# zendesk/min-tfs-client

Measured on NVIDIA H100. Metric: TensorProto encode+decode GB/s, higher is better.
Workload: dtype u8

## Files before the change

### min-tfs-client_b200/csrc/codec_host.cpp

```cpp
#include <cuda_runtime.h>
#include <stdarg.h>
#include <stdio.h>
#include <stdlib.h>
#include <string.h>

#include <algorithm>
#include <string>
#include <unordered_map>
#include <vector>

#include "../../include/b200tfs.h"
#include "frame.h"
#include "kernels.h"
#include "plan.h"
#include "tpl.h"
#include "walker.h"
#include "wire.h"

using namespace b200tfs;

static thread_local char g_err[512] = "";

static int fail(int code, const char* fmt, ...) {
  va_list ap;
// ... 1095 lines not shown
        else pb.payload(w + r.off, dst + run, bytes, op, r.len, r.stride);
        run += bytes;
      }
      if (pad) {
        if (run % di.elem_size || run > o.dst_bytes) return fail(B200TFS_E_SHAPE, "output %d: %llu value bytes for a tensor of %llu", j,
                                                                  (unsigned long long)run, (unsigned long long)o.dst_bytes);
        fills.push_back(Fill{dst, di.elem_size, run / di.elem_size, o.n_elems});
      }
    } else {
      if (want != o.dtype) return fail(B200TFS_E_DTYPE, "output %d: cast on varint dtypes is not supported", j);
      VarDecodeJob vj{};
      bool plain = runs.size() <= (size_t)B200TFS_MAX_RUNS;
      for (const b200tfs_run& r : runs) plain = plain && r.count == 1;
      if (plain) {
        vj.n_chunks = (int)runs.size();
        for (size_t k = 0; k < runs.size(); ++k) { vj.src[k] = w + runs[k].off; vj.len[k] = runs[k].len; }
      } else {
        gather_cur = (gather_cur + 15) & ~15ull;
        uint8_t* g = (uint8_t*)c->gather_dev.p + gather_cur;
        uint64_t at = 0;
        for (const b200tfs_run& r : runs) {
          const uint64_t bytes = (uint64_t)r.len * r.count;
          if (r.count == 1) pb.payload(w + r.off, g + at, bytes, OP_COPY);
          else pb.payload(w + r.off, g + at, bytes, OP_COPY, r.len, r.stride);
          at += bytes;
        }
        gather_cur += at;
        vj.n_chunks = 1; vj.src[0] = g; vj.len[0] = at;
      }
      vj.dst = dst; vj.n_elems = o.n_elems; vj.dtype = o.dtype; vj.out_index = j; vj.half_as_value = half_as_value; vj.pad_edge = pad;
      vjobs.push_back(vj);
    }
  }
  int rc = launch_plan(c, pb);
  if (rc) return rc;
  for (const Fill& f : fills) { CU(launch_fill_edge(f.dst, f.elem_size, f.have, nullptr, f.n_elems, c->stream)); c->launches += 1; }
  c->pending_status.clear();
  if (!vjobs.empty()) {
    if ((rc = run_vardecode(c, vjobs, status))) return rc;
  }
  if (status && wait) {
    CU(cudaStreamSynchronize(c->stream));
    collect_varint_status(c, status);
  }
  return B200TFS_OK;
}

extern "C" int b200tfs_unpack_outputs(b200tfs_ctx* c, const void* arena_dev, int32_t m, const b200tfs_output* outs,
                                      const uint64_t* out_rec_off, void* const* dst_dev, const int32_t* dst_dtype, int32_t* status) {
  return unpack_outputs_impl(c, arena_dev, m, outs, out_rec_off, dst_dev, dst_dtype, status, true);
}

namespace {
struct FusedLayout { uint64_t outs, nouts, specs, status, vstatus, total; };
FusedLayout fused_layout(int32_t n) {
  FusedLayout L;
  L.outs = 0;
  L.nouts = L.outs + sizeof(b200tfs_output) * (uint64_t)n * kFusedMaxOutputs;
  L.specs = (L.nouts + 4ull * n + 15) & ~15ull;
  L.status = L.specs + sizeof(b200tfs_model_spec) * (uint64_t)n;
  L.vstatus = (L.status + 4ull * n + 15) & ~15ull;
  L.total = (L.vstatus + 4ull * n * kFusedMaxOutputs + 15) & ~15ull;
  return L;
}

struct VarPlanLayout { uint64_t jobs, segs, tile_seg, tile_val, group_sum, total, status, n_tiles, bytes; };
VarPlanLayout var_plan_layout(uint64_t n, uint64_t tile_cap) {
  const uint64_t slots = n * kFusedMaxOutputs;
  VarPlanLayout V;
  V.jobs = 0;
  V.segs = V.jobs + slots * sizeof(VarJobDev);
  V.tile_seg = (V.segs + slots * B200TFS_MAX_RUNS * sizeof(VarSeg) + 15) & ~15ull;
  V.tile_val = (V.tile_seg + 4 * tile_cap + 15) & ~15ull;
  V.group_sum = (V.tile_val + 4 * tile_cap + 15) & ~15ull;
  V.total = (V.group_sum + 4 * (tile_cap / kVarGroupTiles + slots + 2) + 15) & ~15ull;
  V.status = V.total + 8 * slots;
  V.n_tiles = (V.status + 4 * slots + 15) & ~15ull;
  V.bytes = V.n_tiles + 16;
  return V;
}
}

extern "C" {

static void adopt_pinned_template(b200tfs_ctx* c) {
  if (!c->tpl_pinned) return;
  const TplInline& p = *c->tpl_pinned;
  if (p.head.serial && (int32_t)(p.head.serial - c->tpl_known.head.serial) > 0) c->tpl_known = p;
}

static uint32_t decode_vpt(const b200tfs_ctx* c, int32_t n, const uint64_t* rec_len) {
  uint64_t wire_total = 0;
  for (int i = 0; i < n; ++i) wire_total += rec_len[i];
  return pick_vec_per_tile(c, c->decode_cast ? wire_total / 2 : wire_total, c->decode_cast ? 65536 : 262144);
}

static bool host_template(const uint8_t* rec0, uint64_t len, uint32_t vpt, uint64_t dst_stride, uint32_t serial, uint32_t cast, uint32_t varints,
                          Template* T) {
  T->in.head.valid = 0;
  if (!rec0 || len == 0 || len > 0x7FFFFFFFull) return false;
  b200tfs_output outs[kFusedMaxOutputs + 1];
  b200tfs_model_spec spec;
  int cnt = 0;
  Cursor cur;
  cur_open_host(cur, rec0, (uint32_t)len);
  SpillArea sp{nullptr, 0u, 0u};
  const int st = walk_response(cur, kFusedMaxOutputs, outs, &cnt, &spec, sp);
  if (st != B200TFS_OK) return false;
  const uint64_t used = tpl_layout_outputs(outs, cnt, dst_stride, cast, varints);
  for (int k = 0; k < cnt; ++k) if (outs[k].status == B200TFS_E_SIZE) return false;
  tpl_learn(T, cur, (uint32_t)len, outs, cnt, spec, st, vpt, (used + 255) & ~255ull, serial, cast, varints);
  return T->in.head.valid != 0;
}

int b200tfs_decode_slot_bytes(const void* wire_host, int32_t n, const uint64_t* rec_off, const uint64_t* rec_len, int32_t varints,
// ... 28 lines not shown
};

static int decode_launch(b200tfs_ctx* c, const void* arena_dev, int32_t n, const uint64_t* rec_off, const uint64_t* rec_len, void* dst_dev,
                         uint64_t dst_stride, uint32_t vpt, const Template* host_tpl, const DecodeSlices* sl = nullptr) {
  const uint64_t tile_bytes = 16ull * vpt;
  FusedLayout L = fused_layout(n);
  int rc;
  if ((rc = grow_host(c, c->fused_host, L.total))) return rc;
  uint64_t var_tile_cap = 0;
  if (c->decode_varints) {
    for (int i = 0; i < n; ++i) var_tile_cap += var_record_tile_bound(rec_len[i]);
    if (var_tile_cap > 0x7FFFFFFFull) return fail(B200TFS_E_TOOBIG, "batch needs more than 2^31 varint tiles");
    if ((rc = grow_dev(c, c->vdec_dev, var_plan_layout((uint64_t)n, var_tile_cap).bytes))) return rc;
  }
  if (!c->tpl_dev) {
    if (c->capturing) return fail(B200TFS_E_ARG, "run b200tfs_decode_responses once before capturing it");
    CU(cudaMalloc(&c->tpl_dev, 2 * sizeof(Template) + 64));
    CU(cudaMemsetAsync(c->tpl_dev, 0, 2 * sizeof(Template) + 64, c->stream));
    CU(cudaHostAlloc((void**)&c->tpl_pinned, sizeof(TplInline), cudaHostAllocPortable | cudaHostAllocMapped));
    memset(c->tpl_pinned, 0, sizeof(TplInline));
  }
  FusedParams fp{};
  fp.w = (const uint8_t*)arena_dev; fp.dst = (uint8_t*)dst_dev; fp.dst_stride = dst_stride; fp.n = n; fp.vpt = vpt;
  fp.tpl_read = (const Template*)c->tpl_dev + (c->tpl_flip & 1);
  fp.tpl_write = (Template*)c->tpl_dev + ((c->tpl_flip & 1) ^ 1);
  c->tpl_flip ^= 1;
  fp.tpl_pinned = c->tpl_pinned;
  fp.stats = (unsigned long long*)((uint8_t*)c->tpl_dev + 2 * sizeof(Template));
  if (++c->serial == 0) c->serial = 1;
  fp.serial = c->serial;
  fp.cast = c->decode_cast;
  fp.varints = c->decode_varints;
  fp.tpli.head.valid = 0;
  if (host_tpl && host_tpl->in.head.valid) {
    if (vpt <= kStageVecsHost) {
      Slot* slot;
      if ((rc = claim_slot(c, sizeof(Template), &slot))) return rc;
      memcpy(slot->host.p, host_tpl, sizeof(Template));
      CU(cudaMemcpyAsync((void*)fp.tpl_read, slot->host.p, sizeof(Template), cudaMemcpyHostToDevice, c->stream));
      if (slot->done) { CU(cudaEventRecord(slot->done, c->stream)); slot->pending = true; }
      c->tpl_known = host_tpl->in;
      if (!c->opt_no_inline) fp.tpli = host_tpl->in;
    }
  } else {
    if (!c->capturing && (!c->tpl_event_pending || cudaEventQuery(c->tpl_event) == cudaSuccess)) { c->tpl_event_pending = false; adopt_pinned_template(c); }
    const TplHead& h = c->tpl_known.head;
    if (vpt <= kStageVecsHost && !c->opt_no_inline && h.valid && h.rec_len == rec_len[0] && h.vpt == vpt && h.cast == fp.cast &&
        h.varints == fp.varints && h.dst_need <= dst_stride)
      fp.tpli = c->tpl_known;
  }
  const TplHead& kh = (host_tpl && host_tpl->in.head.valid) ? host_tpl->in.head : c->tpl_known.head;
  const bool budget_known = kh.valid && kh.vpt == vpt && kh.cast == fp.cast && kh.varints == fp.varints && kh.dst_need <= dst_stride;
  auto ctas_for = [&](uint64_t len) -> uint64_t {
    if (budget_known && len == kh.rec_len) return (uint64_t)kh.total_tiles + 2;
    return (len + tile_bytes - 1) / tile_bytes + kFusedSlackTiles;
  };
  uint8_t* d = (uint8_t*)c->fused_host.p;
  fp.outs = (b200tfs_output*)(d + L.outs); fp.n_outs = (int32_t*)(d + L.nouts);
  fp.specs = (b200tfs_model_spec*)(d + L.specs); fp.status = (int32_t*)(d + L.status);
  auto lay_out = [&](FusedParams& q, auto&& per, uint64_t* grid_out) -> int {
    uint64_t grid = 0;
    if (n <= kFusedInlineRecs) {
      for (int i = 0; i < n; ++i) {
        q.inl.off[i] = rec_off[i]; q.inl.len[i] = rec_len[i]; q.inl.tile_start[i] = (uint32_t)grid;
        grid += per(rec_len[i]);
      }
      q.inl.tile_start[n] = (uint32_t)grid;
    } else {
      std::vector<uint32_t> ts(n + 1);
      for (int i = 0; i < n; ++i) { ts[i] = (uint32_t)grid; grid += per(rec_len[i]); }
      ts[n] = (uint32_t)grid;
      if (grid > 0x7FFFFFFFull) return fail(B200TFS_E_TOOBIG, "batch needs more than 2^31 tiles");
      const uint64_t o_ts = (grid * 4 + 15) & ~15ull, o_off = (o_ts + 4ull * (n + 1) + 15) & ~15ull, o_len = o_off + 8ull * n;
      const uint64_t image = o_len + 8ull * n;
      Slot* slot;
      int rc2;
      if ((rc2 = claim_slot(c, image, &slot))) return rc2;
      uint8_t* h = (uint8_t*)slot->host.p;
      uint32_t* cr = (uint32_t*)h;
      for (int i = 0; i < n; ++i) for (uint32_t t = ts[i]; t < ts[i + 1]; ++t) cr[t] = (uint32_t)i;
      memcpy(h + o_ts, ts.data(), 4ull * (n + 1));
      memcpy(h + o_off, rec_off, 8ull * n);
      memcpy(h + o_len, rec_len, 8ull * n);
      if ((rc2 = upload_slot(c, slot, image))) return rc2;
      uint8_t* sd = (uint8_t*)slot->dev.p;
      q.cta_rec = (const uint32_t*)sd; q.tile_start = (const uint32_t*)(sd + o_ts);
      q.rec_off = (const uint64_t*)(sd + o_off); q.rec_len = (const uint64_t*)(sd + o_len);
    }
    if (grid > 0x7FFFFFFFull) return fail(B200TFS_E_TOOBIG, "batch needs more than 2^31 tiles");
    *grid_out = grid;
    return B200TFS_OK;
  };
  const TplInline* kt = (host_tpl && host_tpl->in.head.valid) ? &host_tpl->in : &c->tpl_known;
  bool split = fp.cast && !sl && budget_known && kh.total_tiles > 0 && (uint64_t)n * kh.rec_len >= (4ull << 20) && !c->opt_no_inline;
  for (int i = 0; i < n && split; ++i) split = rec_len[i] == kh.rec_len;
  if (split) {
    if ((rc = grow_dev(c, c->guard_dev, 4ull * n))) return rc;
    FusedParams fa = fp;
    fa.mode = 1; fa.guard = (uint32_t*)c->guard_dev.p; fa.tpli = *kt;
    uint64_t ga = 0;
    if ((rc = lay_out(fa, [](uint64_t) -> uint64_t { return 2; }, &ga))) return rc;
    CU(launch_decode_fused(fa, (uint32_t)ga, c->stream));
    PlanBuilder pb;
    uint32_t per_rec = 0;
    for (uint32_t q = 0; q < kt->head.n_chunks; ++q) if (kt->chunk[q].n_tiles) ++per_rec;
    pb.items.reserve((size_t)n * per_rec);
    for (int i = 0; i < n; ++i)
      for (uint32_t q = 0; q < kt->head.n_chunks; ++q) {
        const TplChunk& ch = kt->chunk[q];
        if (!ch.n_tiles) continue;
        const bool narrow = ch.op == OP_F2H || ch.op == OP_F2B;
        const uint64_t n_out = narrow ? ch.len / 2 : ch.len;
        pb.items.push_back(MoveItem{(const uint8_t*)arena_dev + rec_off[i] + ch.wire_off, (uint8_t*)dst_dev + (uint64_t)i * dst_stride + ch.dst_off, n_out,
                                    ch.op, 0, 0, 0});
        pb.large_bytes += n_out;
      }
    pb.guard = (const uint32_t*)c->guard_dev.p; pb.guard_div = per_rec;
    BuiltPlan bp;
    if ((rc = build_plan(c, pb, true, &bp))) return rc;
    CU(launch_move_guarded(bp.plan_dev, bp.ph.n_tiles, c->stream));
    if (bp.slot && bp.slot->done && !c->capturing) { CU(cudaEventRecord(bp.slot->done, c->stream)); bp.slot->pending = true; }
    c->launches += 2;
    fp.mode = 2; fp.guard = (uint32_t*)c->guard_dev.p;
  }
  uint64_t grid = 0;
  if ((rc = lay_out(fp, ctas_for, &grid))) return rc;
  if (sl) {
    if (n != 1 || !fp.tpli.head.valid) return fail(B200TFS_E_ARG, "internal: sliced decode without a host template");
    fp.trusted = 1;
    for (int k = 0; k < sl->K; ++k) {
      CU(cudaStreamWaitEvent(c->stream, sl->before[k], 0));
      fp.tile_bias = sl->tile_lo[k];
      const uint32_t end = (k + 1 == sl->K) ? (uint32_t)grid : sl->tile_lo[k + 1];
      CU(launch_decode_fused(fp, end - sl->tile_lo[k], c->stream));
      CU(cudaEventRecord(sl->after[k], c->stream));
      c->launches += 1;
    }
  } else {
    CU(launch_decode_fused(fp, (uint32_t)grid, c->stream));
    c->launches += 1;
  }
  c->fused_varints = fp.varints != 0;
  if (fp.varints) {
    const VarPlanLayout V = var_plan_layout((uint64_t)n, var_tile_cap);
    uint8_t* vd = (uint8_t*)c->vdec_dev.p;
    VarPlan vp{};
    vp.outs = fp.outs; vp.n_outs = fp.n_outs; vp.rec_status = fp.status;
    vp.w = fp.w; vp.rec_off = fp.rec_off;
    if (n <= kFusedInlineRecs) for (int i = 0; i < n; ++i) vp.off_inl[i] = rec_off[i];
    vp.dst = fp.dst; vp.dst_stride = dst_stride; vp.n = (uint32_t)n; vp.tile_cap = (uint32_t)var_tile_cap;
    vp.jobs = (VarJobDev*)(vd + V.jobs); vp.segs = (VarSeg*)(vd + V.segs); vp.tile_seg = (uint32_t*)(vd + V.tile_seg);
    vp.tile_val = (uint32_t*)(vd + V.tile_val); vp.group_sum = (uint32_t*)(vd + V.group_sum);
    vp.total = (unsigned long long*)(vd + V.total); vp.status = (int32_t*)(vd + V.status); vp.n_tiles = (uint32_t*)(vd + V.n_tiles);
    CU(launch_vdec_plan(vp, c->stream));
    VarTables tb{};
    tb.segs = vp.segs; tb.tile_seg = vp.tile_seg; tb.jobs = vp.jobs; tb.n_tiles = vp.tile_cap; tb.n_tiles_dev = vp.n_tiles;
    CU(launch_vdec_dev(tb, (uint32_t)c->sm_count * 4, c->stream));
    CU(cudaMemcpyAsync((uint8_t*)c->fused_host.p + L.vstatus, vp.status, 4ull * n * kFusedMaxOutputs, cudaMemcpyDeviceToHost, c->stream));
    c->launches += 3;
  }
  c->fused_n = n;
  if (!c->capturing) { CU(cudaEventRecord(c->tpl_event, c->stream)); c->tpl_event_pending = true; }
  return B200TFS_OK;
}

int b200tfs_decode_responses(b200tfs_ctx* c, const void* arena_dev, int32_t n, const uint64_t* rec_off, const uint64_t* rec_len,
                             void* dst_dev, uint64_t dst_stride) {
  if (!c || n < 0 || (n && (!arena_dev || !rec_off || !rec_len || !dst_dev))) return fail(B200TFS_E_ARG, "bad arguments");
  if (n == 0) return B200TFS_OK;
  if (dst_stride & 255) return fail(B200TFS_E_ARG, "dst_stride must be a multiple of 256");
  if (!c->capturing) CU(cudaSetDevice(c->device));
  return decode_launch(c, arena_dev, n, rec_off, rec_len, dst_dev, dst_stride, decode_vpt(c, n, rec_len), nullptr);
}

int b200tfs_set_decode_cast(b200tfs_ctx* c, int32_t float_as) {
  if (!c) return fail(B200TFS_E_ARG, "ctx is NULL");
  if (c->capturing) return fail(B200TFS_E_ARG, "cannot change the decode cast during graph capture");
  if (float_as != 0 && float_as != DT_FLOAT && float_as != DT_HALF && float_as != DT_BFLOAT16)
    return fail(B200TFS_E_DTYPE, "DT_FLOAT outputs can leave as DT_FLOAT, DT_HALF or DT_BFLOAT16, not as dtype %d", float_as);
  c->decode_cast = (float_as == DT_HALF || float_as == DT_BFLOAT16) ? (uint32_t)float_as : 0u;
  return B200TFS_OK;
}

int b200tfs_set_decode_varints(b200tfs_ctx* c, int32_t on) {
  if (!c) return fail(B200TFS_E_ARG, "ctx is NULL");
  if (c->capturing) return fail(B200TFS_E_ARG, "cannot switch the varint decode during graph capture");
  c->decode_varints = on ? 1u : 0u;
  return B200TFS_OK;
}

int b200tfs_decode_results(b200tfs_ctx* c, int32_t n, b200tfs_output* outs, int32_t* n_outs, b200tfs_model_spec* specs,
                           int32_t* rec_status) {
  if (!c || n < 0) return fail(B200TFS_E_ARG, "bad arguments");
  if (c->capturing) return fail(B200TFS_E_ARG, "cannot collect results during graph capture");
  if (n > c->fused_n) return fail(B200TFS_E_ARG, "only %d records were decoded", c->fused_n);
  FusedLayout L = fused_layout(c->fused_n);
  CU(cudaStreamSynchronize(c->stream));
  const uint8_t* h = (const uint8_t*)c->fused_host.p;
  if (outs) memcpy(outs, h + L.outs, sizeof(b200tfs_output) * (uint64_t)n * kFusedMaxOutputs);
  if (outs && c->fused_varints) {
    const int32_t* rs = (const int32_t*)(h + L.status);
    const int32_t* no = (const int32_t*)(h + L.nouts);
    const int32_t* vs = (const int32_t*)(h + L.vstatus);
    for (int r = 0; r < n; ++r)
      for (int k = 0; k < no[r] && rs[r] == B200TFS_OK && k < kFusedMaxOutputs; ++k) {
        b200tfs_output& o = outs[(size_t)r * kFusedMaxOutputs + k];
        const int32_t s = vs[(size_t)r * kFusedMaxOutputs + k];
        if (s == kVarSlotIdle) continue;
        o.status = s;
        o.flags |= B200TFS_OF_DEVICE_VARINT;
      }
  }
  if (n_outs) memcpy(n_outs, h + L.nouts, 4ull * n);
  if (specs) memcpy(specs, h + L.specs, sizeof(b200tfs_model_spec) * (uint64_t)n);
  if (rec_status) memcpy(rec_status, h + L.status, 4ull * n);
  return B200TFS_OK;
}

int b200tfs_decode_stats(b200tfs_ctx* c, uint64_t* param_template, uint64_t* device_template, uint64_t* walked) {
  if (!c) return fail(B200TFS_E_ARG, "ctx is NULL");
  if (c->capturing) return fail(B200TFS_E_ARG, "cannot read the counters during graph capture");
  unsigned long long v[3] = {0, 0, 0};
  if (c->tpl_dev) {
    CU(cudaSetDevice(c->device));
    CU(cudaMemcpyAsync(v, (uint8_t*)c->tpl_dev + 2 * sizeof(Template), sizeof v, cudaMemcpyDeviceToHost, c->stream));
    CU(cudaStreamSynchronize(c->stream));
  }
  if (param_template) *param_template = v[0];
  if (device_template) *device_template = v[1];
  if (walked) *walked = v[2];
  return B200TFS_OK;
}

int b200tfs_capture_begin(b200tfs_ctx* c) {
  if (!c) return fail(B200TFS_E_ARG, "ctx is NULL");
  if (c->capturing) return fail(B200TFS_E_ARG, "already capturing");
  CU(cudaSetDevice(c->device));
  CU(cudaStreamSynchronize(c->stream));
  adopt_pinned_template(c);
  for (auto& s : c->slots) s.pending = false;
  CU(cudaStreamBeginCapture(c->stream, cudaStreamCaptureModeRelaxed));
  c->capturing = true;
  return B200TFS_OK;
}

int b200tfs_capture_end(b200tfs_ctx* c, void** graph_exec) {
  if (!c || !graph_exec) return fail(B200TFS_E_ARG, "NULL argument");
  if (!c->capturing) return fail(B200TFS_E_ARG, "not capturing");
  c->capturing = false;
  cudaGraph_t g = nullptr;
  CU(cudaStreamEndCapture(c->stream, &g));
  cudaGraphExec_t ge = nullptr;
  cudaError_t e = cudaGraphInstantiate(&ge, g, 0);
  cudaGraphDestroy(g);
  if (e != cudaSuccess) return fail(B200TFS_E_CUDA, "cudaGraphInstantiate: %s", cudaGetErrorString(e));
  c->has_graphs = true;
  *graph_exec = ge;
  return B200TFS_OK;
}

int b200tfs_graph_launch(b200tfs_ctx* c, void* graph_exec) {
  if (!c || !graph_exec) return fail(B200TFS_E_ARG, "NULL argument");
  CU(cudaGraphLaunch((cudaGraphExec_t)graph_exec, c->stream));
  return B200TFS_OK;
}

int b200tfs_graph_destroy(void* graph_exec) {
// ... 675 lines not shown
```

### min-tfs-client_b200/csrc/kernels.cu

```cuda
#include <cuda_bf16.h>
#include <cuda_fp16.h>
#include <cuda_runtime.h>
#include <stdint.h>
#include <stdlib.h>
#include <string.h>

#include <algorithm>
#include <utility>

#include "frame.h"
#include "kernels.h"
#include "plan.h"
#include "tpl.h"
#include "walker.h"
#include "wire.h"

namespace b200tfs {

__device__ __forceinline__ uint4 ld_stream(const uint8_t* p) {
  uint4 r;
  asm volatile("ld.global.nc.L1::no_allocate.v4.u32 {%0,%1,%2,%3}, [%4];"
               : "=r"(r.x), "=r"(r.y), "=r"(r.z), "=r"(r.w) : "l"(p));
  return r;
}
// ... 608 lines not shown
  const uint64_t* s = reinterpret_cast<const uint64_t*>(src);
  uint64_t* d = reinterpret_cast<uint64_t*>(dst);
  for (uint32_t i = threadIdx.x; i < bytes / 8; i += blockDim.x) d[i] = s[i];
}

__device__ __noinline__ void fused_slow_path(const FusedParams& fp, uint32_t r, uint32_t j, uint32_t budget, bool publish, const uint8_t* rec,
                                             uint64_t len, uint8_t* dst_slot, uint8_t* lines, b200tfs_output* outs_s, b200tfs_model_spec& spec_s,
                                             FusedJob& job) {
    int cnt = 0, st;
    Cursor c;
    job.valid = 0;
    if (len > 0x7FFFFFFFull) st = B200TFS_E_PARSE;
    else {
      cur_open(c, rec, (uint32_t)len, lines);
      SpillArea sp{nullptr, 0u, 0u};
      st = walk_response(c, kFusedMaxOutputs, outs_s, &cnt, &spec_s, sp);
      if (st == B200TFS_E_SPILL) st = B200TFS_E_NONCANONICAL;
    }
    uint64_t cursor = 0;
    uint32_t t_base = 0;
    if (st == B200TFS_OK) {
      cursor = tpl_layout_outputs(outs_s, cnt, fp.dst_stride, fp.cast, fp.varints);
      uint32_t done_mask[kFusedMaxOutputs] = {0};
      for (;;) {
        int bk = -1, bq = -1; uint64_t best = ~0ull;
        for (int k = 0; k < cnt; ++k) {
          const b200tfs_output& o = outs_s[k];
          if (o.status != B200TFS_OK || !o.n_elems || dtype_info(o.dtype).kind != VK_FIXED) continue;
          for (int q = 0; q < o.n_runs; ++q)
            if (!(done_mask[k] >> q & 1) && o.runs[q].off < best) { best = o.runs[q].off; bk = k; bq = q; }
        }
        if (bk < 0) break;
        done_mask[bk] |= 1u << bq;
        const b200tfs_output& o = outs_s[bk];
        uint64_t run = 0;
        for (int q = 0; q < bq; ++q) run += (uint64_t)o.runs[q].len * o.runs[q].count;
        const b200tfs_run& rn = o.runs[bq];
        const bool narrow = tpl_narrows(fp.cast, o.dtype);
        const uint64_t bytes = ((uint64_t)rn.len * rn.count) >> (narrow ? 1 : 0);
        const uint32_t nt = tiles_for(bytes, fp.vpt);
        if (j >= t_base && j < t_base + nt) {
          job.src = rec + rn.off; job.dst = dst_slot + o.dst_off + (narrow ? run / 2 : run); job.n_out = bytes;
          job.op = tpl_move_op(fp.cast, o.dtype); job.n_tiles = nt; job.tile = j - t_base; job.valid = 1;
          job.glen = rn.count > 1 ? rn.len : 0u; job.gstride = rn.count > 1 ? rn.stride : 0u;
        }
        t_base += nt;
      }
      if (t_base > budget) st = B200TFS_E_NONCANONICAL;
    }
    if (publish) {
      if (fp.stats) atomicAdd(&fp.stats[2], 1ull);
      fp.status[r] = st;
      fp.n_outs[r] = (st == B200TFS_OK) ? cnt : 0;
      fp.specs[r] = spec_s;
      for (int k = 0; k < cnt && st == B200TFS_OK; ++k) fp.outs[(size_t)r * kFusedMaxOutputs + k] = outs_s[k];
      if (r == 0) {
        if (len <= 0x7FFFFFFFull) tpl_learn(fp.tpl_write, c, (uint32_t)len, outs_s, cnt, spec_s, st, fp.vpt, (cursor + 255) & ~255ull, fp.serial, fp.cast,
                                            fp.varints);
        else fp.tpl_write->in.head.valid = 0;
        if (fp.tpl_pinned) {
          fp.tpl_pinned->head.valid = 0;
          __threadfence_system();
          const uint64_t* s8 = reinterpret_cast<const uint64_t*>(&fp.tpl_write->in);
          uint64_t* d8 = reinterpret_cast<uint64_t*>(fp.tpl_pinned);
          const bool ok = fp.tpl_write->in.head.valid != 0;
          if (ok) for (uint32_t q = sizeof(TplHead) / 8; q < sizeof(TplInline) / 8; ++q) d8[q] = s8[q];
          __threadfence_system();
          TplHead h = fp.tpl_write->in.head;
          h.serial = fp.serial; h.valid = ok ? 1u : 0u;
          const uint64_t* h8 = reinterpret_cast<const uint64_t*>(&h);
          for (uint32_t q = sizeof(TplHead) / 8; q-- > 0;) d8[q] = h8[q];
        }
      }
    }
    if (st != B200TFS_OK) job.valid = 0;
}

template <bool STAGED, bool CAST>
__device__ __forceinline__ void decode_fused_body(const FusedParams& fp) {
  pdl_launch_dependents();
  __shared__ __align__(16) uint8_t lines[256];
  __shared__ b200tfs_output outs_s[kFusedMaxOutputs + 1];
  __shared__ b200tfs_model_spec spec_s;
  __shared__ FusedJob job;
  extern __shared__ __align__(128) uint8_t stage_smem[];
  __shared__ __align__(8) uint64_t stage_bars[kStageBufs];
  __shared__ TplChunk ch_s[kTplChunks];
  __shared__ TplHead th_s;
  if (STAGED && threadIdx.x == 0) {
    for (uint32_t q = 0; q < kStageBufs; ++q) mbar_init(&stage_bars[q], 1);
    asm volatile("fence.mbarrier_init.release.cluster;" ::: "memory");
  }
  const uint32_t b = blockIdx.x + fp.tile_bias;
  uint32_t r, j, budget;
  uint64_t off, len;
  if (fp.n <= kFusedInlineRecs) {
    r = 0;
    while (r + 1 < (uint32_t)fp.n && b >= fp.inl.tile_start[r + 1]) ++r;
    j = b - fp.inl.tile_start[r]; off = fp.inl.off[r]; len = fp.inl.len[r];
    budget = fp.inl.tile_start[r + 1] - fp.inl.tile_start[r];
  } else {
    r = fp.cta_rec[b];
    const uint32_t t0 = fp.tile_start[r];
    j = b - t0; off = fp.rec_off[r]; len = fp.rec_len[r];
    budget = fp.tile_start[r + 1] - t0;
  }
  const uint8_t* rec = fp.w + off;
  uint8_t* dst_slot = fp.dst + (uint64_t)r * fp.dst_stride;
  pdl_wait_prior_grids();
  if (CAST && fp.mode == 2 && fp.guard[r] != 0) return;

  const Template* T = fp.tpl_read;
  const bool inl = !STAGED && fp.tpli.head.valid != 0;
  uint32_t live = budget;
  const uint32_t i = threadIdx.x;
  {
    if (inl) {
      if (i < kTplChunks) ch_s[i] = fp.tpli.chunk[i];
      if (i == kTplChunks) th_s = fp.tpli.head;
    } else {
      if (i < kTplChunks) ch_s[i] = T->in.chunk[i];
      if (i == kTplChunks) th_s = T->in.head;
    }
    __syncthreads();
    const uint32_t nch = th_s.n_chunks;
    if (th_s.valid && th_s.rec_len == len && th_s.vpt == fp.vpt && th_s.cast == fp.cast && th_s.varints == fp.varints && th_s.dst_need <= fp.dst_stride &&
        (th_s.total_tiles < budget || (CAST && fp.mode == 1))) {
      auto verdict = [&]() -> bool {
        bool same = true;
        if (!STAGED && fp.trusted && inl) return true;
        if (STAGED) {
          if (i < th_s.framing_len) {
            uint32_t w = i;
            for (uint32_t q = 0; q < nch; ++q) if (ch_s[q].fpos <= i) w += ch_s[q].len;
            same = rec[w] == T->in.framing[i];
          }
          if (i < nch && ch_s[i].is_varint && ch_s[i].len) same = same && !(rec[ch_s[i].wire_off + ch_s[i].len - 1] & 0x80);
          return __syncthreads_and(same) != 0;
        }
        const uint32_t lane = i & 31;
        for (uint32_t k = lane; k < th_s.framing_len; k += 32) {
          uint32_t w = k;
          for (uint32_t q = 0; q < nch; ++q) if (ch_s[q].fpos <= k) w += ch_s[q].len;
          const uint8_t want = inl ? fp.tpli.framing[k] : T->in.framing[k];
          same = same && rec[w] == want;
        }
        if (lane < nch && ch_s[lane].is_varint && ch_s[lane].len) same = same && !(rec[ch_s[lane].wire_off + ch_s[lane].len - 1] & 0x80);
        return __all_sync(0xFFFFFFFFu, same) != 0;
      };
      uint32_t t_base = 0, mine = kTplChunks;
      for (uint32_t q = 0; q < nch; ++q) {
        const uint32_t nt = ch_s[q].n_tiles;
        if (j >= t_base && j < t_base + nt) { mine = q; break; }
        t_base += nt;
      }
      if (CAST && fp.mode == 1) {
        mine = kTplChunks;
        const bool ok = verdict();
        if (j == 0) { if (threadIdx.x == 0) fp.guard[r] = ok ? 1u : 0u; return; }
        if (!ok) return;
      }
      if (mine == kTplChunks && j != 0 && j != budget - 1) return;
      live = max(th_s.total_tiles, 1u);
      bool hit;
      if (STAGED) {
        StagedTile stg{};
        const bool narrow = CAST && mine < kTplChunks && op_narrows(ch_s[mine].op);
        if (mine < kTplChunks && !narrow)
          stg = staged_begin(rec + ch_s[mine].wire_off, dst_slot + ch_s[mine].dst_off, ch_s[mine].len, ch_s[mine].op, j - t_base, fp.vpt,
                             stage_smem, stage_bars);
        if (narrow)
          hit = move_tile<false>(rec + ch_s[mine].wire_off, dst_slot + ch_s[mine].dst_off, (uint64_t)(ch_s[mine].len >> 1), ch_s[mine].op,
                                 ch_s[mine].n_tiles, j - t_base, fp.vpt, verdict);
        else hit = verdict();
        if (hit && mine < kTplChunks && !narrow) {
          if (stg.use)
            staged_finish(stg, rec + ch_s[mine].wire_off, dst_slot + ch_s[mine].dst_off, ch_s[mine].len, ch_s[mine].op, ch_s[mine].n_tiles,
                          j - t_base, stage_smem, stage_bars);
          else
            move_tile_cold(rec + ch_s[mine].wire_off, dst_slot + ch_s[mine].dst_off, ch_s[mine].len, ch_s[mine].op, ch_s[mine].n_tiles, j - t_base,
                           fp.vpt);
        }
        if (!hit) staged_drain(stg, stage_bars, 0);
      } else if (CAST && mine < kTplChunks && op_narrows(ch_s[mine].op)) {
        hit = move_tile<false>(rec + ch_s[mine].wire_off, dst_slot + ch_s[mine].dst_off, (uint64_t)(ch_s[mine].len >> 1), ch_s[mine].op,
                               ch_s[mine].n_tiles, j - t_base, fp.vpt, verdict);
      } else if (mine < kTplChunks) {
        hit = move_tile<true>(rec + ch_s[mine].wire_off, dst_slot + ch_s[mine].dst_off, ch_s[mine].len, ch_s[mine].op, ch_s[mine].n_tiles,
                              j - t_base, fp.vpt, verdict);
      } else hit = verdict();
      if (hit) {
        if (j == budget - 1) {
          const bool table_ok = !inl || (T->in.head.valid && T->in.head.serial == th_s.serial);
          if (table_ok) {
            if (threadIdx.x == 0 && fp.stats) atomicAdd(&fp.stats[inl ? 0 : 1], 1ull);
            publish_words(fp.outs + (size_t)r * kFusedMaxOutputs, T->outs, th_s.n_outs * (uint32_t)sizeof(b200tfs_output));
            publish_words(fp.specs + r, &T->spec, (uint32_t)sizeof(b200tfs_model_spec));
            if (threadIdx.x == 0) { fp.status[r] = B200TFS_OK; fp.n_outs[r] = (int32_t)th_s.n_outs; }
            if (r == 0) publish_words(fp.tpl_write, T, (uint32_t)sizeof(Template));
          } else if (threadIdx.x == 0) {
            fused_slow_path(fp, r, 0, budget, true, rec, len, dst_slot, lines, outs_s, spec_s, job);
          }
        }
        return;
      }
    }
  }

  if (CAST && fp.mode == 1) { if (j == 0 && threadIdx.x == 0) fp.guard[r] = 0u; return; }
  if (threadIdx.x == 0) fused_slow_path(fp, r, j, live, j == 0, rec, len, dst_slot, lines, outs_s, spec_s, job);
  __syncthreads();
  if (job.valid) {
    if (job.gstride) move_tile_gather(SrcView{job.src, job.glen, job.gstride}, job.dst, job.n_out, job.op, job.n_tiles, job.tile, fp.vpt);
    else if (CAST && op_narrows(job.op)) move_tile_narrow(job.src, job.dst, job.n_out, job.op, job.n_tiles, job.tile, fp.vpt);
    else move_tile_cold(job.src, job.dst, job.n_out, job.op, job.n_tiles, job.tile, fp.vpt);
  }
}

__global__ void __launch_bounds__(kMoveThreads, 2) decode_fused_kernel(const __grid_constant__ FusedParams fp) { decode_fused_body<false, false>(fp); }
__global__ void __launch_bounds__(kMoveThreads, 2) decode_fused_staged_kernel(const __grid_constant__ FusedParams fp) { decode_fused_body<true, false>(fp); }
__global__ void __launch_bounds__(kMoveThreads, 2) decode_fused_cast_kernel(const __grid_constant__ FusedParams fp) { decode_fused_body<false, true>(fp); }
__global__ void __launch_bounds__(kMoveThreads, 2) decode_fused_staged_cast_kernel(const __grid_constant__ FusedParams fp) { decode_fused_body<true, true>(fp); }

#include "varint_kernels.cuh"

__device__ __forceinline__ uint64_t concat_scan(uint64_t v, uint64_t& carry, unsigned long long* warp_sum) {
  const uint32_t lane = threadIdx.x & 31, wid = threadIdx.x >> 5;
  uint64_t inc = v;
#pragma unroll
  for (int d = 1; d < 32; d <<= 1) {
    const uint64_t x = __shfl_up_sync(0xFFFFFFFFu, inc, d);
    if (lane >= (uint32_t)d) inc += x;
  }
  if (lane == 31) warp_sum[wid] = inc;
  __syncthreads();
  uint64_t before = carry, round = 0;
  for (uint32_t w = 0; w < kConcatPlanThreads / 32; ++w) {
    const uint64_t x = warp_sum[w];
    if (w < wid) before += x;
    round += x;
  }
  __syncthreads();
  carry += round;
  return before + inc - v;
}

__global__ void __launch_bounds__(kConcatPlanThreads) concat_plan_kernel(const __grid_constant__ ConcatPlan cp) {
  __shared__ unsigned long long warp_sum[kConcatPlanThreads / 32];
  __shared__ uint32_t ref_rec;
  const uint32_t n = cp.n, nk = cp.n_keys;
  MoveItem* items = reinterpret_cast<MoveItem*>(cp.plan + ((sizeof(PlanHeader) + 15) & ~15ull));
// ... 296 lines not shown
```

### min-tfs-client_b200/csrc/plan.h

```cpp
#pragma once
#include <stdint.h>

#include "../../include/b200tfs.h"

namespace b200tfs {

enum MoveOp : uint32_t {
  OP_COPY = 0,
  OP_QUIET_SRC = 1,
  OP_QUIET_DST = 2,
  OP_BOOL = 3,
  OP_H2F = 4,
  OP_B2F = 5,
  OP_F2H = 6,
  OP_F2B = 7,
  OP_FLAG_BLOB = 0x80000000u
};

struct MoveItem {
  const uint8_t* src;
  uint8_t* dst;
  uint64_t n_out;
  uint32_t op;
  uint32_t n_tiles;
// ... 3 lines not shown
struct TileRef { uint32_t item; uint32_t tile; };

struct SmallItem {
  uint64_t src;
  uint8_t* dst;
  uint32_t n_out;
  uint32_t op;
  uint32_t glen, gstride;
};

struct PlanHeader {
  uint32_t n_items, n_tiles, n_small, uniform_tpi;
  uint32_t vec_per_tile;
  uint32_t off_items, off_tiles, off_small;
  uint32_t guard_div;
  uint32_t independent;
  uint32_t pad[2];
  const uint32_t* guard;
};

constexpr uint32_t kInlinePlanBytes = 3840;
struct InlinePlan { uint8_t bytes[kInlinePlanBytes]; };

constexpr uint32_t kMoveThreads = 256;
constexpr uint32_t kSmallMax = 2048;

constexpr int kFusedMaxOutputs = 8;
constexpr int kFusedInlineRecs = 16;
constexpr uint32_t kFusedSlackTiles = 8;

struct FusedInline { uint64_t off[kFusedInlineRecs], len[kFusedInlineRecs]; uint32_t tile_start[kFusedInlineRecs + 1]; };

constexpr uint32_t kTplChunks = 4;
constexpr uint32_t kTplFraming = 256;
struct TplChunk { uint32_t wire_off, len, dst_off, op, n_tiles, is_varint, fpos, pad; };
struct TplHead {
  uint32_t valid, n_chunks, n_outs, framing_len;
  uint64_t rec_len, dst_need;
  uint32_t vpt, total_tiles;
  uint32_t serial, cast;
  uint32_t varints, pad;
};
struct TplInline {
  TplHead head;
  TplChunk chunk[kTplChunks];
  uint8_t framing[kTplFraming];
};
struct Template {
  TplInline in;
  b200tfs_model_spec spec;
  b200tfs_output outs[kFusedMaxOutputs];
};

struct FusedParams {
  const uint8_t* w;
  uint8_t* dst;
  uint64_t dst_stride;
  int32_t n;
  uint32_t vpt;
  b200tfs_output* outs;
  int32_t* n_outs;
  b200tfs_model_spec* specs;
  int32_t* status;
  const uint32_t* cta_rec;
  const uint32_t* tile_start;
  const uint64_t* rec_off;
  const uint64_t* rec_len;
  const Template* tpl_read;
  Template* tpl_write;
  TplInline* tpl_pinned;
  unsigned long long* stats;
  uint32_t serial;
  uint32_t cast;
  uint32_t mode;
  uint32_t* guard;
  uint32_t tile_bias;
  uint32_t trusted;
  uint32_t varints;
  uint32_t pad;
  FusedInline inl;
  TplInline tpli;
};

constexpr uint32_t kVarThreads = 256;
constexpr uint32_t kVarPerThread = 8;
constexpr uint32_t kVarTileElems = kVarThreads * kVarPerThread;
constexpr uint32_t kVarTileBytes = kVarThreads * 32;
constexpr int32_t kVarFlagHalfAsValue = 1;
constexpr int32_t kVarFlagPadEdge = 2;

struct VarSeg {
  const uint8_t* src;
  uint64_t n;
  uint32_t job;
  uint32_t first_tile;
};

constexpr uint32_t kVarGroupTiles = kVarThreads;

struct VarJobDev {
  uint8_t* dst;
  uint64_t n_elems;
  uint64_t cap;
  uint32_t* tile_val;
  uint32_t* group_sum;
  unsigned long long* total;
  int32_t* status;
  int32_t dtype;
  uint32_t elem_size;
  uint32_t is_signed;
  int32_t flags;
  uint32_t first_tile;
  uint32_t n_tiles;
  uint32_t pad[2];
};

struct VarTables {
  const VarSeg* segs;
  const uint32_t* tile_seg;
  const VarJobDev* jobs;
  uint32_t n_tiles;
  uint32_t single;
  VarSeg seg0;
  VarJobDev job0;
  const uint32_t* n_tiles_dev;
};

constexpr uint32_t kVarPlanThreads = 1024;
constexpr int32_t kVarSlotIdle = 1;
struct VarPlan {
  const b200tfs_output* outs;
  const int32_t* n_outs;
  const int32_t* rec_status;
  const uint8_t* w;
  const uint64_t* rec_off;
  uint64_t off_inl[kFusedInlineRecs];
  uint8_t* dst;
  uint64_t dst_stride;
  uint32_t n, tile_cap;
  VarJobDev* jobs;
  VarSeg* segs;
  uint32_t* tile_seg;
  uint32_t* tile_val;
  uint32_t* group_sum;
  unsigned long long* total;
  int32_t* status;
  uint32_t* n_tiles;
};
constexpr uint64_t var_record_tile_bound(uint64_t len) { return len / kVarTileBytes + 2 + 2ull * kFusedMaxOutputs * B200TFS_MAX_RUNS; }

constexpr uint32_t kConcatPlanThreads = 1024;
struct ConcatKeyDev { const uint8_t* key; uint8_t* dst; uint64_t cap; uint32_t key_len, pad; };
struct ConcatPlan {
  const uint8_t* w;
  const uint64_t* rec_off;
  const b200tfs_output* outs;
  const int32_t* n_outs;
  const int32_t* rec_status;
  const ConcatKeyDev* keys;
  uint32_t n, n_keys, out_stride, cast;
  uint32_t vpt, tile_cap;
  int32_t* kst;
  int32_t* match;
  uint8_t* plan;
  b200tfs_output* vouts;
  int32_t* vn_outs;
  int32_t* vrec_status;
};
constexpr uint64_t concat_record_tile_bound(uint64_t len, uint64_t tile_bytes, uint32_t n_keys) {
  return len / tile_bytes + 1ull + (uint64_t)n_keys * B200TFS_MAX_RUNS;
}

enum FrameSegKind : uint32_t {
  FS_BYTES = 0,
  FS_VARINT = 1,
  FS_BE32 = 2,
  FS_ITEM = 3,
  FS_SMALL = 4,
  FS_VARJOB = 5,
  FS_TINYVAR = 6
};
constexpr uint32_t kTinyVarElems = 32;
struct TinyVar { const uint8_t* src; uint32_t n, elem_size, is_signed, pad; };
struct FrameSeg { uint32_t kind, a, b, pad; };
enum FrameTermKind : uint32_t { FT_TOTAL = 0, FT_VAL = 1, FT_VLEN = 2, FT_TINY = 3 };
struct FrameTerm { uint32_t kind, idx; };
// ... 34 lines not shown
```

### min-tfs-client_b200/csrc/varint_kernels.cuh

```cuda

__device__ __forceinline__ uint32_t bitsel(uint32_t m, uint32_t a, uint32_t b) {
  uint32_t d;
  asm("lop3.b32 %0, %1, %2, %3, 0xE4;" : "=r"(d) : "r"(a), "r"(b), "r"(m));
  return d;
}

__device__ __forceinline__ uint32_t vlen64(uint64_t v) {
  const uint32_t nb = 64u - (uint32_t)__clzll((long long)(v | 1ull));
  return ((nb + 6u) * 37u) >> 8;
}

template <uint32_t SZ, bool SG>
__device__ __forceinline__ uint64_t ldg_elem(const uint8_t* p) {
  if (SZ == 1) { const uint8_t t = __ldg(p); return SG ? (uint64_t)(int64_t)(int8_t)t : t; }
  if (SZ == 2) { const uint16_t t = __ldg(reinterpret_cast<const uint16_t*>(p)); return SG ? (uint64_t)(int64_t)(int16_t)t : t; }
  if (SZ == 4) { const uint32_t t = __ldg(reinterpret_cast<const uint32_t*>(p)); return SG ? (uint64_t)(int64_t)(int32_t)t : t; }
  return __ldg(reinterpret_cast<const unsigned long long*>(p));
}

template <uint32_t SZ, bool SG>
__device__ __forceinline__ void load_striped_t(const uint8_t* src, uint64_t e0, uint32_t cnt, uint64_t (&v)[kVarPerThread]) {
  const uint8_t* base = src + (e0 + threadIdx.x) * SZ;
  if (cnt == kVarTileElems) {
#pragma unroll
// ... 414 lines not shown
  const uint32_t packed = __popc(startm[0]) | (__popc(startm[1]) << 16);
  uint32_t packed_total;
  uint64_t before;
  const uint32_t rank = block_scan_sum(packed, &packed_total, share, &before, sh);
  const uint32_t first_total = packed_total & 0xFFFFu, n_here = first_total + (packed_total >> 16);
#pragma unroll
  for (uint32_t r = 0; r < 2; ++r) {
    uint32_t starts = startm[r], at = (r == 0) ? (rank & 0xFFFFu) : first_total + (rank >> 16);
    const uint32_t at0 = 16 * (threadIdx.x + r * kVarThreads + 1);
    while (starts) {
      const uint32_t i = __ffs(starts) - 1;
      starts &= starts - 1;
      start_at[at++] = (uint16_t)(at0 + i);
    }
  }
  __syncthreads();
  const uint64_t idx0 = before + (smraw[15] >> 7);
  if (threadIdx.x == 0 && hi > G && hi <= G + kVarTileBytes && (hi[-1] & 0x80)) atomicMin(jb.status, B200TFS_E_PARSE);
  int32_t st_local;
  switch (jb.dtype) {
    case DT_INT64: case DT_UINT64: st_local = decode_elems<VS_U64>(smraw, start_at, n_here, jb.dst, idx0, n_store); break;
    case DT_INT32: case DT_UINT32: st_local = decode_elems<VS_U32>(smraw, start_at, n_here, jb.dst, idx0, n_store); break;
    case DT_INT16: st_local = decode_elems<VS_I16>(smraw, start_at, n_here, jb.dst, idx0, n_store); break;
    case DT_INT8: st_local = decode_elems<VS_I8>(smraw, start_at, n_here, jb.dst, idx0, n_store); break;
    case DT_UINT16: st_local = decode_elems<VS_U16>(smraw, start_at, n_here, jb.dst, idx0, n_store); break;
    case DT_UINT8: st_local = decode_elems<VS_U8>(smraw, start_at, n_here, jb.dst, idx0, n_store); break;
    case DT_BOOL: st_local = decode_elems<VS_BOOL>(smraw, start_at, n_here, jb.dst, idx0, n_store); break;
    case DT_HALF: case DT_BFLOAT16:
      st_local = (jb.flags & kVarFlagHalfAsValue) ? decode_elems<VS_HALF_VALUE>(smraw, start_at, n_here, jb.dst, idx0, n_store)
                                                  : decode_elems<VS_HALF_BITS>(smraw, start_at, n_here, jb.dst, idx0, n_store);
      break;
    default: st_local = B200TFS_OK; break;
  }
  if (st_local != B200TFS_OK) atomicMin(jb.status, st_local);
}
__global__ void __launch_bounds__(kVarThreads) vdec_emit_kernel(const __grid_constant__ VarTables tb) { vdec_emit_tile(tb, blockIdx.x); }
__global__ void __launch_bounds__(kVarThreads) vdec_emit_dev_kernel(const __grid_constant__ VarTables tb) {
  const uint32_t nt = *tb.n_tiles_dev;
  for (uint32_t t = blockIdx.x; t < nt; t += gridDim.x) {
    vdec_emit_tile(tb, t);
    __syncthreads();
  }
}

__global__ void __launch_bounds__(kVarPlanThreads) vdec_plan_kernel(const __grid_constant__ VarPlan vp) {
  __shared__ unsigned long long warp_sum[kVarPlanThreads / 32];
  const uint32_t lane = threadIdx.x & 31, wid = threadIdx.x >> 5;
  const uint32_t slots = vp.n * (uint32_t)kFusedMaxOutputs;
  unsigned long long carry = 0;
  for (uint32_t s0 = 0; s0 < slots; s0 += kVarPlanThreads) {
    const uint32_t s = s0 + threadIdx.x, r = s / kFusedMaxOutputs, k = s % kFusedMaxOutputs;
    int32_t st = kVarSlotIdle;
    uint32_t tiles = 0, n_runs = 0;
    const b200tfs_output* o = vp.outs + s;
    const uint8_t* rec = nullptr;
    if (s < slots && vp.rec_status[r] == B200TFS_OK && (int32_t)k < vp.n_outs[r] && o->status == B200TFS_OK && o->n_elems &&
        (dtype_info(o->dtype).kind == VK_VARINT || dtype_info(o->dtype).kind == VK_BOOL)) {
      rec = vp.w + (vp.n <= (uint32_t)kFusedInlineRecs ? vp.off_inl[r] : vp.rec_off[r]);
      n_runs = (uint32_t)o->n_runs;
      st = B200TFS_OK;
      if ((o->flags & (B200TFS_OF_UNPACKED | B200TFS_OF_SPILLED)) || o->n_inline != n_runs || n_runs > B200TFS_MAX_RUNS) st = B200TFS_E_NONCANONICAL;
      for (uint32_t q = 0; q < n_runs && st == B200TFS_OK; ++q) {
        if (o->runs[q].count != 1) st = B200TFS_E_NONCANONICAL;
        else tiles += (uint32_t)var_decode_tiles(rec + o->runs[q].off, o->runs[q].len);
      }
      if (st != B200TFS_OK) { tiles = 0; n_runs = 0; }
    }
    const uint32_t groups = (tiles + kVarGroupTiles - 1) / kVarGroupTiles;
    const unsigned long long v = (unsigned long long)tiles | ((unsigned long long)groups << 32);
    unsigned long long inc = v;
#pragma unroll
    for (int d = 1; d < 32; d <<= 1) {
      const unsigned long long x = __shfl_up_sync(0xFFFFFFFFu, inc, d);
      if (lane >= (uint32_t)d) inc += x;
    }
    if (lane == 31) warp_sum[wid] = inc;
    __syncthreads();
    unsigned long long before = carry, round = 0;
    for (uint32_t w = 0; w < kVarPlanThreads / 32; ++w) {
      const unsigned long long x = warp_sum[w];
      if (w < wid) before += x;
      round += x;
    }
    __syncthreads();
    before += inc - v;
    carry += round;
    const uint32_t first_tile = (uint32_t)before, first_group = (uint32_t)(before >> 32);
    const bool over = st == B200TFS_OK && first_tile + tiles > vp.tile_cap;
    if (s < slots) {
      vp.status[s] = over ? B200TFS_E_NONCANONICAL : st;
      vp.total[s] = 0;
      VarJobDev jb{};
      if (st == B200TFS_OK) {
        jb.dst = vp.dst + (uint64_t)r * vp.dst_stride + o->dst_off;
        jb.n_elems = over ? ~0ull : o->n_elems;
        jb.dtype = o->dtype;
        jb.elem_size = dtype_info(o->dtype).elem_size;
        jb.is_signed = dtype_info(o->dtype).is_signed;
        jb.first_tile = first_tile;
        jb.n_tiles = tiles;
        jb.tile_val = vp.tile_val + first_tile;
        jb.group_sum = vp.group_sum + first_group;
        jb.total = vp.total + s;
        jb.status = vp.status + s;
        const uint32_t run_tiles = over ? vp.tile_cap - min(first_tile, vp.tile_cap) : tiles;
        for (uint32_t g = 0; g < (run_tiles + kVarGroupTiles - 1) / kVarGroupTiles; ++g) jb.group_sum[g] = 0;
        uint32_t t = first_tile;
// ... 15 lines not shown
```

Before: 1450.

## Publish shared template outputs once per launch instead of per record

When records match a cached template, the fused decode kernel stops writing the full output and spec tables for every record. It writes one shared template table from an extra CTA and stores only a per-record serial reference. The host expands these references after sync, and the varint planner reads the shared table through them. Single-tile records also get a budget of one CTA instead of total+2, which trims idle CTAs. The cost is an extra CTA, host-side memcpy expansion, and more bookkeeping that could go out of sync between components.

After: 1451, median of 6. No clear change (+0.0%).

```diff
diff --git a/min-tfs-client_b200/csrc/codec_host.cpp b/min-tfs-client_b200/csrc/codec_host.cpp
--- a/min-tfs-client_b200/csrc/codec_host.cpp
+++ b/min-tfs-client_b200/csrc/codec_host.cpp
@@ -1171,7 +1171,7 @@
 }
 
 namespace {
-struct FusedLayout { uint64_t outs, nouts, specs, status, vstatus, total; };
+struct FusedLayout { uint64_t outs, nouts, specs, status, vstatus, tpl_ref, tpl_table, total; };
 FusedLayout fused_layout(int32_t n) {
   FusedLayout L;
   L.outs = 0;
@@ -1179,7 +1179,9 @@
   L.specs = (L.nouts + 4ull * n + 15) & ~15ull;
   L.status = L.specs + sizeof(b200tfs_model_spec) * (uint64_t)n;
   L.vstatus = (L.status + 4ull * n + 15) & ~15ull;
-  L.total = (L.vstatus + 4ull * n * kFusedMaxOutputs + 15) & ~15ull;
+  L.tpl_ref = (L.vstatus + 4ull * n * kFusedMaxOutputs + 15) & ~15ull;
+  L.tpl_table = (L.tpl_ref + 4ull * n + 15) & ~15ull;
+  L.total = (L.tpl_table + sizeof(FusedTplTable) + 15) & ~15ull;
   return L;
 }
 
@@ -1314,12 +1316,14 @@
   const TplHead& kh = (host_tpl && host_tpl->in.head.valid) ? host_tpl->in.head : c->tpl_known.head;
   const bool budget_known = kh.valid && kh.vpt == vpt && kh.cast == fp.cast && kh.varints == fp.varints && kh.dst_need <= dst_stride;
   auto ctas_for = [&](uint64_t len) -> uint64_t {
+    if (fp.tpli.head.valid && len == fp.tpli.head.rec_len && fp.tpli.head.total_tiles <= 1) return 1;
     if (budget_known && len == kh.rec_len) return (uint64_t)kh.total_tiles + 2;
     return (len + tile_bytes - 1) / tile_bytes + kFusedSlackTiles;
   };
   uint8_t* d = (uint8_t*)c->fused_host.p;
   fp.outs = (b200tfs_output*)(d + L.outs); fp.n_outs = (int32_t*)(d + L.nouts);
   fp.specs = (b200tfs_model_spec*)(d + L.specs); fp.status = (int32_t*)(d + L.status);
+  fp.tpl_ref = (uint32_t*)(d + L.tpl_ref); fp.tpl_table = (FusedTplTable*)(d + L.tpl_table);
   auto lay_out = [&](FusedParams& q, auto&& per, uint64_t* grid_out) -> int {
     uint64_t grid = 0;
     if (n <= kFusedInlineRecs) {
@@ -1350,7 +1354,8 @@
       q.rec_off = (const uint64_t*)(sd + o_off); q.rec_len = (const uint64_t*)(sd + o_len);
     }
     if (grid > 0x7FFFFFFFull) return fail(B200TFS_E_TOOBIG, "batch needs more than 2^31 tiles");
-    *grid_out = grid;
+    q.tpl_table_cta = n > 1 ? (uint32_t)grid : ~0u;
+    *grid_out = grid + (n > 1 ? 1 : 0);
     return B200TFS_OK;
   };
   const TplInline* kt = (host_tpl && host_tpl->in.head.valid) ? &host_tpl->in : &c->tpl_known;
@@ -1408,6 +1413,7 @@
     uint8_t* vd = (uint8_t*)c->vdec_dev.p;
     VarPlan vp{};
     vp.outs = fp.outs; vp.n_outs = fp.n_outs; vp.rec_status = fp.status;
+    vp.tpl_ref = fp.tpl_ref; vp.tpl_outs = fp.tpl_table->outs;
     vp.w = fp.w; vp.rec_off = fp.rec_off;
     if (n <= kFusedInlineRecs) for (int i = 0; i < n; ++i) vp.off_inl[i] = rec_off[i];
     vp.dst = fp.dst; vp.dst_stride = dst_stride; vp.n = (uint32_t)n; vp.tile_cap = (uint32_t)var_tile_cap;
@@ -1460,6 +1466,19 @@
   CU(cudaStreamSynchronize(c->stream));
   const uint8_t* h = (const uint8_t*)c->fused_host.p;
   if (outs) memcpy(outs, h + L.outs, sizeof(b200tfs_output) * (uint64_t)n * kFusedMaxOutputs);
+  if (specs) memcpy(specs, h + L.specs, sizeof(b200tfs_model_spec) * (uint64_t)n);
+  {
+    const uint32_t* ref = (const uint32_t*)(h + L.tpl_ref);
+    const FusedTplTable& tt = *(const FusedTplTable*)(h + L.tpl_table);
+    const int32_t* no = (const int32_t*)(h + L.nouts);
+    for (int r = 0; r < n; ++r) {
+      if (!ref[r]) continue;
+      if (ref[r] != tt.serial || no[r] < 0 || no[r] > kFusedMaxOutputs)
+        return fail(B200TFS_E_CUDA, "internal: record %d refers to template %u, the launch published %u", r, ref[r], tt.serial);
+      if (outs) memcpy(outs + (size_t)r * kFusedMaxOutputs, tt.outs, sizeof(b200tfs_output) * (size_t)no[r]);
+      if (specs) specs[r] = tt.spec;
+    }
+  }
   if (outs && c->fused_varints) {
     const int32_t* rs = (const int32_t*)(h + L.status);
     const int32_t* no = (const int32_t*)(h + L.nouts);
@@ -1474,7 +1493,6 @@
       }
   }
   if (n_outs) memcpy(n_outs, h + L.nouts, 4ull * n);
-  if (specs) memcpy(specs, h + L.specs, sizeof(b200tfs_model_spec) * (uint64_t)n);
   if (rec_status) memcpy(rec_status, h + L.status, 4ull * n);
   return B200TFS_OK;
 }
diff --git a/min-tfs-client_b200/csrc/kernels.cu b/min-tfs-client_b200/csrc/kernels.cu
--- a/min-tfs-client_b200/csrc/kernels.cu
+++ b/min-tfs-client_b200/csrc/kernels.cu
@@ -684,6 +684,7 @@
       if (fp.stats) atomicAdd(&fp.stats[2], 1ull);
       fp.status[r] = st;
       fp.n_outs[r] = (st == B200TFS_OK) ? cnt : 0;
+      fp.tpl_ref[r] = 0u;
       fp.specs[r] = spec_s;
       for (int k = 0; k < cnt && st == B200TFS_OK; ++k) fp.outs[(size_t)r * kFusedMaxOutputs + k] = outs_s[k];
       if (r == 0) {
@@ -724,6 +725,17 @@
     asm volatile("fence.mbarrier_init.release.cluster;" ::: "memory");
   }
   const uint32_t b = blockIdx.x + fp.tile_bias;
+  if (b == fp.tpl_table_cta) {
+    pdl_wait_prior_grids();
+    const Template* T = fp.tpl_read;
+    const uint32_t valid = T->in.head.valid, serial = T->in.head.serial, n_outs = min(T->in.head.n_outs, (uint32_t)kFusedMaxOutputs);
+    if (valid) {
+      publish_words(fp.tpl_table->outs, T->outs, n_outs * (uint32_t)sizeof(b200tfs_output));
+      publish_words(&fp.tpl_table->spec, &T->spec, (uint32_t)sizeof(b200tfs_model_spec));
+    }
+    if (threadIdx.x == 0) fp.tpl_table->serial = valid ? serial : 0u;
+    return;
+  }
   uint32_t r, j, budget;
   uint64_t off, len;
   if (fp.n <= kFusedInlineRecs) {
@@ -757,7 +769,7 @@
     __syncthreads();
     const uint32_t nch = th_s.n_chunks;
     if (th_s.valid && th_s.rec_len == len && th_s.vpt == fp.vpt && th_s.cast == fp.cast && th_s.varints == fp.varints && th_s.dst_need <= fp.dst_stride &&
-        (th_s.total_tiles < budget || (CAST && fp.mode == 1))) {
+        (th_s.total_tiles <= budget || (CAST && fp.mode == 1))) {
       auto verdict = [&]() -> bool {
         bool same = true;
         if (!STAGED && fp.trusted && inl) return true;
@@ -825,10 +837,15 @@
         if (j == budget - 1) {
           const bool table_ok = !inl || (T->in.head.valid && T->in.head.serial == th_s.serial);
           if (table_ok) {
-            if (threadIdx.x == 0 && fp.stats) atomicAdd(&fp.stats[inl ? 0 : 1], 1ull);
-            publish_words(fp.outs + (size_t)r * kFusedMaxOutputs, T->outs, th_s.n_outs * (uint32_t)sizeof(b200tfs_output));
-            publish_words(fp.specs + r, &T->spec, (uint32_t)sizeof(b200tfs_model_spec));
-            if (threadIdx.x == 0) { fp.status[r] = B200TFS_OK; fp.n_outs[r] = (int32_t)th_s.n_outs; }
+            const bool own = fp.tpl_table_cta == ~0u;
+            if (own) {
+              publish_words(fp.outs + (size_t)r * kFusedMaxOutputs, T->outs, th_s.n_outs * (uint32_t)sizeof(b200tfs_output));
+              publish_words(fp.specs + r, &T->spec, (uint32_t)sizeof(b200tfs_model_spec));
+            }
+            if (threadIdx.x == 0) {
+              if (fp.stats) atomicAdd(&fp.stats[inl ? 0 : 1], 1ull);
+              fp.status[r] = B200TFS_OK; fp.n_outs[r] = (int32_t)th_s.n_outs; fp.tpl_ref[r] = own ? 0u : th_s.serial;
+            }
             if (r == 0) publish_words(fp.tpl_write, T, (uint32_t)sizeof(Template));
           } else if (threadIdx.x == 0) {
             fused_slow_path(fp, r, 0, budget, true, rec, len, dst_slot, lines, outs_s, spec_s, job);
diff --git a/min-tfs-client_b200/csrc/plan.h b/min-tfs-client_b200/csrc/plan.h
--- a/min-tfs-client_b200/csrc/plan.h
+++ b/min-tfs-client_b200/csrc/plan.h
@@ -79,6 +79,12 @@
   b200tfs_output outs[kFusedMaxOutputs];
 };
 
+struct FusedTplTable {
+  uint32_t serial, pad;
+  b200tfs_model_spec spec;
+  b200tfs_output outs[kFusedMaxOutputs];
+};
+
 struct FusedParams {
   const uint8_t* w;
   uint8_t* dst;
@@ -89,6 +95,10 @@
   int32_t* n_outs;
   b200tfs_model_spec* specs;
   int32_t* status;
+  uint32_t* tpl_ref;
+  FusedTplTable* tpl_table;
+  uint32_t tpl_table_cta;
+  uint32_t pad0;
   const uint32_t* cta_rec;
   const uint32_t* tile_start;
   const uint64_t* rec_off;
@@ -159,6 +169,8 @@
   const b200tfs_output* outs;
   const int32_t* n_outs;
   const int32_t* rec_status;
+  const uint32_t* tpl_ref;
+  const b200tfs_output* tpl_outs;
   const uint8_t* w;
   const uint64_t* rec_off;
   uint64_t off_inl[kFusedInlineRecs];
diff --git a/min-tfs-client_b200/csrc/varint_kernels.cuh b/min-tfs-client_b200/csrc/varint_kernels.cuh
--- a/min-tfs-client_b200/csrc/varint_kernels.cuh
+++ b/min-tfs-client_b200/csrc/varint_kernels.cuh
@@ -490,7 +490,7 @@
     const uint32_t s = s0 + threadIdx.x, r = s / kFusedMaxOutputs, k = s % kFusedMaxOutputs;
     int32_t st = kVarSlotIdle;
     uint32_t tiles = 0, n_runs = 0;
-    const b200tfs_output* o = vp.outs + s;
+    const b200tfs_output* o = (s < slots && vp.tpl_ref && vp.tpl_ref[r]) ? vp.tpl_outs + k : vp.outs + s;
     const uint8_t* rec = nullptr;
     if (s < slots && vp.rec_status[r] == B200TFS_OK && (int32_t)k < vp.n_outs[r] && o->status == B200TFS_OK && o->n_elems &&
         (dtype_info(o->dtype).kind == VK_VARINT || dtype_info(o->dtype).kind == VK_BOOL)) {
```
